# izhengfan/se2lam

Hardware: NVIDIA H100
Metric: ORB keypoints/sec at 640x480 (8-level pyramid, 1000 kps/frame) (higher is better)
Workload: dtype u8

## Files before the change

### se2lam_b200/csrc/fast_screen.h

```cpp
#pragma once
#include <cstdint>

#if defined(__CUDACC__)
#define SE2_HD __host__ __device__ __forceinline__
#else
#define SE2_HD inline
#endif

namespace fastpx {
SE2_HD int16_t lo16(unsigned a) { return (int16_t)(a & 0xFFFF); }
SE2_HD int16_t hi16(unsigned a) { return (int16_t)(a >> 16); }
SE2_HD unsigned pack16(int lo, int hi) { return ((unsigned)lo & 0xFFFFu) | ((unsigned)hi << 16); }
SE2_HD unsigned perm(unsigned a, unsigned b, unsigned s) {
#if defined(__CUDA_ARCH__)
    return __byte_perm(a, b, s);
#else
    const uint64_t src = ((uint64_t)b << 32) | a;
    unsigned r = 0;
    for (int i = 0; i < 4; ++i) {
        const unsigned sel = (s >> (4 * i)) & 0xF;
        unsigned byte = (unsigned)(src >> (8 * (sel & 7))) & 0xFF;
        if (sel & 8) byte = (byte & 0x80) ? 0xFF : 0x00;
        r |= byte << (8 * i);
    }
    return r;
#endif
}
SE2_HD unsigned maxs2(unsigned a, unsigned b) {
#if defined(__CUDA_ARCH__)
    return __vmaxs2(a, b);
#else
    return pack16(lo16(a) > lo16(b) ? lo16(a) : lo16(b), hi16(a) > hi16(b) ? hi16(a) : hi16(b));
#endif
}
SE2_HD unsigned mins2(unsigned a, unsigned b) {
#if defined(__CUDA_ARCH__)
    return __vmins2(a, b);
#else
    return pack16(lo16(a) < lo16(b) ? lo16(a) : lo16(b), hi16(a) < hi16(b) ? hi16(a) : hi16(b));
#endif
}
SE2_HD unsigned min3s2(unsigned a, unsigned b, unsigned c) {
#if defined(__CUDA_ARCH__)
    return __vimin3_s16x2(a, b, c);
#else
    return mins2(mins2(a, b), c);
#endif
}
SE2_HD unsigned max3s2(unsigned a, unsigned b, unsigned c) {
#if defined(__CUDA_ARCH__)
    return __vimax3_s16x2(a, b, c);
#else
    return maxs2(maxs2(a, b), c);
#endif
}
SE2_HD unsigned add2(unsigned a, unsigned b) {
#if defined(__CUDA_ARCH__)
    return __vadd2(a, b);
#else
    return pack16((lo16(a) + lo16(b)) & 0xFFFF, (hi16(a) + hi16(b)) & 0xFFFF);
#endif
}
}

namespace fastpx {

SE2_HD unsigned screen_T1(int t) { return (unsigned)(0x10000 - (257 + t)) * 0x10001u; }
SE2_HD unsigned screen_U1(int t) { return (unsigned)(256 - t) * 0x10001u; }

SE2_HD unsigned screen4(unsigned n3, unsigned s3, unsigned n2l, unsigned n2c, unsigned n2r, unsigned s2l, unsigned s2c, unsigned s2r,
                        unsigned zl, unsigned zc, unsigned zr, unsigned T1, unsigned U1) {
    const unsigned w_m3 = perm(zl, zc, 0x4321), w_p3 = perm(zc, zr, 0x6543);
    const unsigned nw_ = perm(n2l, n2c, 0x5432), ne_ = perm(n2c, n2r, 0x5432);
    const unsigned sw_ = perm(s2l, s2c, 0x5432), se_ = perm(s2c, s2r, 0x5432);
    unsigned m = 0;
#if defined(__CUDA_ARCH__)
#pragma unroll
#endif
    for (int hlf = 0; hlf < 2; ++hlf) {
        const unsigned sel = hlf ? 0x4342u : 0x4140u;
        const unsigned cb = perm(zc, 0, sel) + 0x01000100u;
        const unsigned e0 = cb - perm(s3, 0, sel), e8 = cb - perm(n3, 0, sel);
        const unsigned e4 = cb - perm(w_p3, 0, sel), e12 = cb - perm(w_m3, 0, sel);
        const unsigned e2 = cb - perm(se_, 0, sel), e10 = cb - perm(nw_, 0, sel);
        const unsigned e6 = cb - perm(ne_, 0, sel), e14 = cb - perm(sw_, 0, sel);
        const unsigned D = mins2(min3s2(maxs2(e0, e8), maxs2(e4, e12), maxs2(e2, e10)), maxs2(e6, e14));
        const unsigned B = maxs2(max3s2(mins2(e0, e8), mins2(e4, e12), mins2(e2, e10)), mins2(e6, e14));
        const unsigned r = maxs2(add2(D, T1), add2(~B, U1));
        const unsigned ok = ~r & 0x80008000u;
        m |= ((ok >> 15) & 1u) << (2 * hlf) | ((ok >> 31) & 1u) << (2 * hlf + 1);
    }
    return m;
}

SE2_HD unsigned inside_mask8(int x0, int cw) {
    const int lo = x0 < 0 ? -x0 : 0;
    const int hi = cw - x0 < 8 ? cw - x0 : 8;
    return (0xFFu << lo) & (0xFFu >> (8 - hi)) & 0xFFu;
}

SE2_HD int first_group(int shift) { return (shift + 3) >> 2; }
SE2_HD int groups_per_row(int cw, int shift) { return ((shift + 2 + cw) >> 2) - first_group(shift) + 1; }
SE2_HD int group_x0(int g, int shift) { return 4 * (g + first_group(shift)) - 3 - shift; }
struct ItemWalk {
    int y, g, dY, dG, G;
    SE2_HD void init(int tid, int nthreads, int groups) { G = groups; y = tid / G; g = tid - y * G; dY = nthreads / G; dG = nthreads - dY * G; }
    SE2_HD void next() { g += dG; y += dY; if (g >= G) { g -= G; ++y; } }
};

constexpr int NMS_X0 = 4;
SE2_HD int nms_plane_bytes(int pw, int ch) { return pw * (ch + 2) + 32; }
SE2_HD int nms_words_per_row(int cw) { return (cw + 31) >> 5; }
SE2_HD unsigned nms_row_mask(int k, int cw) { const int n = cw - 32 * k; return n >= 32 ? 0xFFFFFFFFu : (1u << n) - 1u; }

SE2_HD unsigned nms32(const uint32_t* u, const uint32_t* c, const uint32_t* d) {
    unsigned c3e[10], c3o[10];
    unsigned r[4];
#if defined(__CUDA_ARCH__)
#pragma unroll
#endif
    for (int j = 0; j < 10; ++j) {
        const unsigned ua = u[j], ca = c[j], da = d[j];
        if (j > 0) c3e[j] = max3s2(perm(ua, 0, 0x4240), perm(ca, 0, 0x4240), perm(da, 0, 0x4240));
        if (j < 9) c3o[j] = max3s2(perm(ua, 0, 0x4341), perm(ca, 0, 0x4341), perm(da, 0, 0x4341));
    }
#if defined(__CUDA_ARCH__)
#pragma unroll
#endif
    for (int g = 0; g < 8; ++g) {
        const int j = g + 1;
        const unsigned ua = u[j], ca = c[j], da = d[j];
        const unsigned ce = perm(ca, 0, 0x4240), co = perm(ca, 0, 0x4341);
        const unsigned ve = maxs2(perm(ua, 0, 0x4240), perm(da, 0, 0x4240));
        const unsigned vo = maxs2(perm(ua, 0, 0x4341), perm(da, 0, 0x4341));
        const unsigned ne = max3s2(perm(c3o[j - 1], c3o[j], 0x5432), ve, c3o[j]);
        const unsigned no = max3s2(c3e[j], vo, perm(c3e[j], c3e[j + 1], 0x5432));
        const unsigned te = ce + 0x00FF00FFu - ne, to = co + 0x00FF00FFu - no;
        const unsigned bytes = perm(te, to, 0x7351);
        if (g & 1) {
            r[g >> 1] = (r[g >> 1] + (bytes << 4)) * 0x01020408u;
        } else {
            r[g >> 1] = bytes;
        }
    }
    return perm(perm(r[0], r[1], 0x7373), perm(r[2], r[3], 0x7373), 0x5410);
}

struct WordRun {
    int w, w1, y, k, wpr;
    SE2_HD void init(int tid, int nthreads, int ch, int words_per_row) {
        wpr = words_per_row;
        const int nw = ch * wpr, q = (nw + nthreads - 1) / nthreads;
        w = tid * q < nw ? tid * q : nw;
        w1 = w + q < nw ? w + q : nw;
        y = w / wpr; k = w - y * wpr;
    }
    SE2_HD bool more() const { return w < w1; }
    SE2_HD void next() { ++w; if (++k == wpr) { k = 0; ++y; } }
};

}
```

### se2lam_b200/csrc/orb.cu

```cuda
#include <cuda.h>

#include <algorithm>
#include <cmath>
#include <cstring>
#include <type_traits>
#include <vector>

#include "blur_px.h"
#include "common.h"
#include "fast_screen.h"
#include "introselect.h"
#include "resp_key.h"

namespace {

using se2gpu::fail;

constexpr int EDGE = 16;
constexpr int HALF_PATCH = 15;
constexpr int PATCH = 31;
constexpr int MAX_LEVELS = 16;
constexpr int FAST_THREADS = 256;
constexpr int ORB_LANES = 4;
constexpr int BLUR_WARPS = 4;
// ... 24 lines not shown
    int skipped;
    int cand_off, cand_cap;
};

struct TileGeo { int level, strip, cg; };

struct CellHdr { int n_base, n_a, n_b, pad; };

struct OrbDev {
    int nlevels, nfeatures, fast_th, t_lo;
    int n_cells, n_tiles;
    const LevelGeo* levels;
    const CellGeo* cells;
    const TileGeo* tiles;
    const int* itab;
    const short* stab;
    uint8_t* plain;
    uint8_t* blurred;
    size_t frame_plane_bytes;
    uint32_t* cand;
    size_t cand_total;
    CellHdr* hdr;
    uint32_t* lkp;
    int lkp_total;
    int* lcount;
    int* err;
    int frame0;
};

__device__ __forceinline__ int reflect101(int p, int len) {
    if (len == 1) return 0;
    while (p < 0 || p >= len) p = p < 0 ? -p : 2 * (len - 1) - p;
    return p;
}

constexpr int PYR0_ROWS = 4;
__global__ void __launch_bounds__(256) orb_pyr0(OrbDev d, LevelGeo L, const uint8_t* __restrict__ imgs, int stride, size_t frame_stride, int nvec) {
    const int tid = threadIdx.y * 64 + threadIdx.x;
    const int f = blockIdx.z + d.frame0;
    const uint8_t* img = imgs + f * frame_stride;
    uint8_t* plane = d.plain + f * d.frame_plane_bytes + L.plane_off;
    const int rows = L.h + 2 * EDGE;
    if (blockIdx.x + 1 < gridDim.x) {
        const int vx = blockIdx.x * 64 + threadIdx.x;
        const int y0 = (blockIdx.y * 4 + threadIdx.y) * PYR0_ROWS;
        if (vx >= nvec) return;
        uint4 v[PYR0_ROWS];
#pragma unroll
        for (int k = 0; k < PYR0_ROWS; ++k)
            if (y0 + k < rows) v[k] = __ldg(reinterpret_cast<const uint4*>(img + (size_t)reflect101(y0 + k - EDGE, L.h) * stride) + vx);
#pragma unroll
        for (int k = 0; k < PYR0_ROWS; ++k)
            if (y0 + k < rows) *reinterpret_cast<uint4*>(plane + (size_t)(y0 + k) * L.pitch + EDGE + 16 * vx) = v[k];
        return;
    }
    const int tail0 = EDGE + 16 * nvec, nw = 4 + (L.pitch - tail0) / 4;
    for (int item = tid; item < 4 * PYR0_ROWS * nw; item += 256) {
        const int r = item / nw, wi = item - r * nw;
        const int y = blockIdx.y * 4 * PYR0_ROWS + r;
        if (y >= rows) break;
        const int x0 = wi < 4 ? 4 * wi : tail0 + 4 * (wi - 4);
        const uint8_t* row = img + (size_t)reflect101(y - EDGE, L.h) * stride;
        uint32_t word = 0;
#pragma unroll
        for (int q = 0; q < 4; ++q) {
            const int x = x0 + q;
            const uint32_t px = (x < L.w + 2 * EDGE) ? row[reflect101(x - EDGE, L.w)] : 0u;
            word |= px << (8 * q);
        }
        *reinterpret_cast<uint32_t*>(plane + (size_t)y * L.pitch + x0) = word;
    }
}

__global__ void __launch_bounds__(128) orb_pyr0_undistort(OrbDev d, LevelGeo L, const uint8_t* __restrict__ imgs, int stride, size_t frame_stride,
                                                          const short2* __restrict__ m1, const uint16_t* __restrict__ m2) {
    const int x4 = (blockIdx.x * 128 + threadIdx.x) * 4, y = blockIdx.y;
    const int f = blockIdx.z + d.frame0;
    if (x4 >= L.pitch) return;
    const uint8_t* img = imgs + f * frame_stride;
    const int dy = reflect101(y - EDGE, L.h);
    uint32_t word = 0;
#pragma unroll
    for (int q = 0; q < 4; ++q) {
        const int x = x4 + q;
        uint32_t o = 0;
        if (x < L.w + 2 * EDGE) {
            const int idx = dy * L.w + reflect101(x - EDGE, L.w);
            const short2 s = __ldg(m1 + idx);
            const int fr = __ldg(m2 + idx), a = fr & 31, b = fr >> 5;
            const int sx = s.x, sy = s.y;
            const bool x0 = (unsigned)sx < (unsigned)L.w, x1 = (unsigned)(sx + 1) < (unsigned)L.w;
            const bool y0 = (unsigned)sy < (unsigned)L.h, y1 = (unsigned)(sy + 1) < (unsigned)L.h;
            const uint8_t* p = img + (ptrdiff_t)sy * stride + sx;
            const int t00 = (x0 && y0) ? p[0] : 0, t01 = (x1 && y0) ? p[1] : 0, t10 = (x0 && y1) ? p[stride] : 0, t11 = (x1 && y1) ? p[stride + 1] : 0;
            const int val = t00 * ((32 - a) * (32 - b) * 32) + t01 * (a * (32 - b) * 32) + t10 * ((32 - a) * b * 32) + t11 * (a * b * 32);
            o = (uint32_t)min(max((val + (1 << 14)) >> 15, 0), 255);
        }
        word |= o << (8 * q);
    }
    uint8_t* plane = d.plain + f * d.frame_plane_bytes + L.plane_off;
    *reinterpret_cast<uint32_t*>(plane + (size_t)y * L.pitch + x4) = word;
}

constexpr int RESIZE_TR = 32, RESIZE_TR_TALL = 64;
struct ResizeRow { int s0, s1, b0, b1; };
struct ResizeCol { int sx0, sx1; short a0, a1; int valid; };
template <int RESIZE_TR>
__global__ void __launch_bounds__(256) orb_resize_w(OrbDev d, LevelGeo L, LevelGeo S, int max_rows, int raw_pitch) {
    static_assert(RESIZE_TR % 32 == 0 && RESIZE_TR <= 128, "row terms take one thread per row in warps 4..7");
    asm volatile("griddepcontrol.launch_dependents;" ::: "memory");
    extern __shared__ __align__(16) uint8_t rs_smem[];
    __shared__ ResizeRow rowinfo[RESIZE_TR];
    __shared__ __align__(16) ResizeCol colinfo[128];
    __shared__ int s_lo[RESIZE_TR / 32], s_hi[RESIZE_TR / 32];
    __shared__ int s_cmin[4], s_cmax[4];
    uint16_t* hbuf = reinterpret_cast<uint16_t*>(rs_smem);
    uint8_t* raw = rs_smem + (size_t)max_rows * 128 * sizeof(uint16_t);
    const int tx = threadIdx.x, ty = threadIdx.y, tid = ty * 32 + tx;
    const int x4 = blockIdx.x * 128 + tx * 4, y0 = blockIdx.y * RESIZE_TR;
    const int f = blockIdx.z + d.frame0;
    const int W = L.w + 2 * EDGE, H = L.h + 2 * EDGE;
    const int* xofs = d.itab + L.tab_off;
    const int* yofs = xofs + L.w;
    const short2* ialpha = reinterpret_cast<const short2*>(d.stab + 2 * (size_t)L.tab_off);
    const short2* ibeta = ialpha + L.w;
    if (tid < 128) {
        const int x = blockIdx.x * 128 + tid;
        ResizeCol c{0, 0, 0, 0, 0};
        int cmin = 0x7fffffff, cmax = -1;
        if (x < W) {
            const int dx = reflect101(x - EDGE, L.w);
            c.sx0 = __ldg(xofs + dx);
            c.sx1 = min(c.sx0 + 1, S.w - 1);
            const short2 aa = __ldg(ialpha + dx);
            c.a0 = aa.x; c.a1 = aa.y; c.valid = 1;
            cmin = c.sx0; cmax = c.sx1;
        }
        colinfo[tid] = c;
#pragma unroll
        for (int o = 16; o > 0; o >>= 1) { cmin = min(cmin, __shfl_xor_sync(0xffffffffu, cmin, o)); cmax = max(cmax, __shfl_xor_sync(0xffffffffu, cmax, o)); }
        if (tx == 0) { s_cmin[ty] = cmin; s_cmax[ty] = cmax; }
    } else if (ty < 4 + RESIZE_TR / 32) {
        const int ry = tid - 128, y = y0 + ry;
        int rmin = 0x7fffffff, rmax = -1;
        if (y < H) {
            const int dy = reflect101(y - EDGE, L.h);
            const int sy = __ldg(yofs + dy);
            const short2 bb = __ldg(ibeta + dy);
            ResizeRow r{min(max(sy, 0), S.h - 1), min(max(sy + 1, 0), S.h - 1), bb.x, bb.y};
            rowinfo[ry] = r;
            rmin = r.s0; rmax = r.s1;
        }
#pragma unroll
        for (int o = 16; o > 0; o >>= 1) { rmin = min(rmin, __shfl_xor_sync(0xffffffffu, rmin, o)); rmax = max(rmax, __shfl_xor_sync(0xffffffffu, rmax, o)); }
        if (tx == 0) { s_lo[ty - 4] = rmin; s_hi[ty - 4] = rmax; }
    }
    __syncthreads();
    const int c_min = min(min(s_cmin[0], s_cmin[1]), min(s_cmin[2], s_cmin[3])), c_max = max(max(s_cmax[0], s_cmax[1]), max(s_cmax[2], s_cmax[3]));
    const int c_lo = c_min & ~15, nvec = c_max < 0 ? 0 : (c_max - c_lo) / 16 + 1;
    int r_lo = s_lo[0], r_hi = s_hi[0];
#pragma unroll
    for (int k = 1; k < RESIZE_TR / 32; ++k) { r_lo = min(r_lo, s_lo[k]); r_hi = max(r_hi, s_hi[k]); }
    const int nsr = r_hi - r_lo + 1;
    if (nsr > max_rows || nvec * 16 > raw_pitch) { if (tid == 0) *d.err = 3; return; }
    const uint8_t* src = d.plain + f * d.frame_plane_bytes + S.plane_off + (size_t)EDGE * S.pitch + EDGE;
    asm volatile("griddepcontrol.wait;" ::: "memory");
    if (nvec <= 16) {
        const int v = tid & 15;
        if (v < nvec)
            for (int r = tid >> 4; r < nsr; r += 16)
                *reinterpret_cast<uint4*>(raw + r * raw_pitch + 16 * v) = __ldg(reinterpret_cast<const uint4*>(src + (size_t)(r_lo + r) * S.pitch + c_lo) + v);
    } else {
        for (int i = tid; i < nsr * nvec; i += 256) {
            const int r = i / nvec, v = i - r * nvec;
            *reinterpret_cast<uint4*>(raw + r * raw_pitch + 16 * v) = __ldg(reinterpret_cast<const uint4*>(src + (size_t)(r_lo + r) * S.pitch + c_lo) + v);
        }
    }
    int sx0[4], sx1[4], a0[4], a1[4];
    unsigned vmask = 0;
#pragma unroll
    for (int q = 0; q < 4; ++q) {
        const ResizeCol c = colinfo[4 * tx + q];
        sx0[q] = c.valid ? c.sx0 - c_lo : 0; sx1[q] = c.valid ? c.sx1 - c_lo : 0;
        a0[q] = c.a0; a1[q] = c.a1;
        vmask |= c.valid ? (0xFFu << (8 * q)) : 0u;
    }
    __syncthreads();
    unsigned wq[4], selq[4];
    bool pairq[4];
    int w0 = 0;
    bool window_ok = true;
    {
        int mn = 0x7fffffff;
#pragma unroll
        for (int q = 0; q < 4; ++q) if ((vmask >> (8 * q)) & 1u) mn = min(mn, sx0[q]);
        if (mn == 0x7fffffff) mn = 0;
        w0 = mn >> 2;
#pragma unroll
        for (int q = 0; q < 4; ++q) {
            const bool valid = (vmask >> (8 * q)) & 1u;
            const int o = valid ? sx0[q] - 4 * w0 : 0;
            if (valid && (o + 1 > 11 || (sx1[q] != sx0[q] + 1 && a1[q] != 0))) window_ok = false;
            pairq[q] = o >= 7;
            const int o2 = o - (pairq[q] ? 4 : 0);
            selq[q] = (unsigned)o2 | ((unsigned)(o2 + 1) << 4);
            wq[q] = ((unsigned)a0[q] & 0xFFFFu) | ((unsigned)a1[q] << 16);
            if (a0[q] < 0 || a1[q] < 0) window_ok = false;
        }
    }
    if (x4 < W) {
        if (window_ok) {
            for (int r = ty; r < nsr; r += 8) {
                const uint32_t* rw = reinterpret_cast<const uint32_t*>(raw + r * raw_pitch) + w0;
                const uint32_t W0 = rw[0], W1 = rw[1], W2 = rw[2];
                unsigned hq[4];
#pragma unroll
                for (int q = 0; q < 4; ++q) {
                    const unsigned bytes = __byte_perm(pairq[q] ? W1 : W0, pairq[q] ? W2 : W1, selq[q]);
                    hq[q] = __dp2a_lo(wq[q], bytes, 0u) >> 4;
                }
                *reinterpret_cast<uint2*>(hbuf + r * 128 + 4 * tx) = make_uint2(hq[0] | (hq[1] << 16), hq[2] | (hq[3] << 16));
            }
        } else {
            for (int r = ty; r < nsr; r += 8) {
                const uint8_t* rp = raw + r * raw_pitch;
                const unsigned h0 = (unsigned)((rp[sx0[0]] * a0[0] + rp[sx1[0]] * a1[0]) >> 4), h1 = (unsigned)((rp[sx0[1]] * a0[1] + rp[sx1[1]] * a1[1]) >> 4);
                const unsigned h2 = (unsigned)((rp[sx0[2]] * a0[2] + rp[sx1[2]] * a1[2]) >> 4), h3 = (unsigned)((rp[sx0[3]] * a0[3] + rp[sx1[3]] * a1[3]) >> 4);
                *reinterpret_cast<uint2*>(hbuf + r * 128 + 4 * tx) = make_uint2((h0 & 0xFFFFu) | (h1 << 16), (h2 & 0xFFFFu) | (h3 << 16));
            }
        }
    }
    __syncthreads();
    if (x4 >= L.pitch) return;
    uint8_t* plane = d.plain + f * d.frame_plane_bytes + L.plane_off;
#pragma unroll
    for (int k = 0; k < RESIZE_TR / 8; ++k) {
        const int r = ty + 8 * k, y = y0 + r;
        if (y >= H) break;
        uint32_t word = 0;
        if (x4 < W) {
            const ResizeRow ri = rowinfo[r];
            const uint2 A = *reinterpret_cast<const uint2*>(hbuf + (ri.s0 - r_lo) * 128 + 4 * tx);
            const uint2 B = *reinterpret_cast<const uint2*>(hbuf + (ri.s1 - r_lo) * 128 + 4 * tx);
            const unsigned v0 = (unsigned)((((ri.b0 * (int)(A.x & 0xFFFFu)) >> 16) + ((ri.b1 * (int)(B.x & 0xFFFFu)) >> 16) + 2) >> 2);
            const unsigned v1 = (unsigned)((((ri.b0 * (int)(A.x >> 16)) >> 16) + ((ri.b1 * (int)(B.x >> 16)) >> 16) + 2) >> 2);
            const unsigned v2 = (unsigned)((((ri.b0 * (int)(A.y & 0xFFFFu)) >> 16) + ((ri.b1 * (int)(B.y & 0xFFFFu)) >> 16) + 2) >> 2);
            const unsigned v3 = (unsigned)((((ri.b0 * (int)(A.y >> 16)) >> 16) + ((ri.b1 * (int)(B.y >> 16)) >> 16) + 2) >> 2);
            word = (v0 | (v1 << 8) | (v2 << 16) | (v3 << 24)) & vmask;
        }
        *reinterpret_cast<uint32_t*>(plane + (size_t)y * L.pitch + x4) = word;
    }
}

__device__ __forceinline__ unsigned fast_cv(int v) { return (unsigned)(256 + v) | ((unsigned)(256 - v) << 16); }
__device__ __forceinline__ unsigned fast_q(unsigned p, unsigned cv) { return p * 0xFFFFu + cv; }

__device__ __forceinline__ int fast_arc_score(const uint8_t* __restrict__ p, int pw) {
    const unsigned cv = fast_cv(p[0]);
    unsigned q[16];
    q[0] = fast_q(p[3 * pw], cv);       q[1] = fast_q(p[3 * pw + 1], cv);   q[2] = fast_q(p[2 * pw + 2], cv);    q[3] = fast_q(p[pw + 3], cv);
    q[4] = fast_q(p[3], cv);            q[5] = fast_q(p[-pw + 3], cv);      q[6] = fast_q(p[-2 * pw + 2], cv);   q[7] = fast_q(p[-3 * pw + 1], cv);
    q[8] = fast_q(p[-3 * pw], cv);      q[9] = fast_q(p[-3 * pw - 1], cv);  q[10] = fast_q(p[-2 * pw - 2], cv);  q[11] = fast_q(p[-pw - 3], cv);
    q[12] = fast_q(p[-3], cv);          q[13] = fast_q(p[pw - 3], cv);      q[14] = fast_q(p[2 * pw - 2], cv);   q[15] = fast_q(p[3 * pw - 1], cv);
    unsigned m3[16];
#pragma unroll
    for (int k = 0; k < 16; ++k) m3[k] = __vimin3_s16x2(q[k], q[(k + 1) & 15], q[(k + 2) & 15]);
    unsigned best = 0;
#pragma unroll
    for (int k = 0; k < 16; k += 2) {
        const unsigned a9 = __vimin3_s16x2(m3[k], m3[(k + 3) & 15], m3[(k + 6) & 15]);
        const unsigned b9 = __vimin3_s16x2(m3[k + 1], m3[(k + 4) & 15], m3[(k + 7) & 15]);
        best = __vimax3_s16x2(best, a9, b9);
    }
    return (int)max(best & 0xFFFFu, best >> 16) - 256;
}

struct FastMaps { CUtensorMap m[MAX_LEVELS]; };
__device__ __forceinline__ unsigned orb_smem_u32(const void* p) { return (unsigned)__cvta_generic_to_shared(p); }
__device__ __forceinline__ void orb_mbar_init(unsigned long long* bar, unsigned count) {
    asm volatile("mbarrier.init.shared::cta.b64 [%0], %1;" ::"r"(orb_smem_u32(bar)), "r"(count) : "memory");
    asm volatile("fence.mbarrier_init.release.cluster;" ::: "memory");
}
__device__ __forceinline__ bool orb_mbar_wait(unsigned long long* bar, unsigned parity) {
    const long long t0 = clock64();
    for (;;) {
        unsigned done;
        asm volatile(
            "{\n"
            ".reg .pred p;\n"
            "mbarrier.try_wait.parity.shared::cta.b64 p, [%1], %2;\n"
            "selp.u32 %0, 1, 0, p;\n"
            "}\n" : "=r"(done) : "r"(orb_smem_u32(bar)), "r"(parity) : "memory");
        if (done) return true;
        if (clock64() - t0 > 400000000LL) return false;
    }
}
__device__ __forceinline__ void orb_tma_box3(void* dst_smem, const CUtensorMap* map, int x, int y, int z, unsigned bytes, unsigned long long* bar) {
    asm volatile("mbarrier.arrive.expect_tx.shared::cta.b64 _, [%0], %1;" ::"r"(orb_smem_u32(bar)), "r"(bytes) : "memory");
    asm volatile("cp.async.bulk.tensor.3d.shared::cluster.global.tile.mbarrier::complete_tx::bytes [%0], [%1, {%2, %3, %4}], [%5];"
                 ::"r"(orb_smem_u32(dst_smem)), "l"(map), "r"(x), "r"(y), "r"(z), "r"(orb_smem_u32(bar)) : "memory");
}

template <bool TMA>
__global__ void __launch_bounds__(FAST_THREADS, TMA ? 0 : 5) orb_fast_cells(OrbDev d, const __grid_constant__ FastMaps maps) {
    extern __shared__ __align__(128) uint8_t smem_raw[];
    __shared__ int s_ncand, s_wsum[FAST_THREADS / 32];
    __shared__ __align__(8) unsigned long long s_bar;
    const CellGeo c = d.cells[blockIdx.x];
    const int f = blockIdx.y + d.frame0;
    CellHdr* hdr = d.hdr + (size_t)f * d.n_cells + blockIdx.x;
    const int cw = c.x1 - c.x0, ch = c.y1 - c.y0;
    if (c.skipped || cw <= 0 || ch <= 0) {
        if (threadIdx.x == 0) { hdr->n_base = 0; hdr->n_a = 0; hdr->n_b = 0; }
        return;
    }
    const LevelGeo& L = d.levels[c.level];
    const int bx0 = c.x0 - 3 + EDGE, ax0 = bx0 & (TMA ? ~15 : ~3), shift = bx0 - ax0;
    const int pw = TMA ? L.fbw : (shift + cw + 6 + 3) & ~3, pww = pw >> 2;
    const int ph = TMA ? L.fbh : ch + 6;
    uint8_t* smem = TMA ? smem_raw + ((128u - (orb_smem_u32(smem_raw) & 127u)) & 127u) : smem_raw;
    const int g0 = fastpx::first_group(shift), G = fastpx::groups_per_row(cw, shift), nitems = ch * G;
    const int wpr = fastpx::nms_words_per_row(cw);
    uint8_t* patch = smem;
    uint8_t* score = smem + ((pw * ph + 15) & ~15);
    uint32_t* bitmap = reinterpret_cast<uint32_t*>(score + ((fastpx::nms_plane_bytes(pw, ch) + 15) & ~15));
    uint16_t* list = reinterpret_cast<uint16_t*>(bitmap + ch * wpr);
    if (TMA) {
        if (threadIdx.x == 0) orb_mbar_init(&s_bar, 1);
        __syncthreads();
        if (threadIdx.x == 0) orb_tma_box3(patch, &maps.m[c.level], ax0, c.y0 - 3 + EDGE, f, (unsigned)(pw * ph), &s_bar);
    } else {
        const uint8_t* plane = d.plain + f * d.frame_plane_bytes + L.plane_off;
        const int by0 = c.y0 - 3 + EDGE;
        for (int i = threadIdx.x; i < pww * ph; i += FAST_THREADS) {
            const int py = i / pww, pxw = i - py * pww;
            reinterpret_cast<uint32_t*>(patch)[i] = *reinterpret_cast<const uint32_t*>(plane + (size_t)(by0 + py) * L.pitch + ax0 + 4 * pxw);
        }
    }
    constexpr int NW = FAST_THREADS / 32;
    const int lane = threadIdx.x & 31, wid = threadIdx.x >> 5;
    const uint8_t* p0 = patch + 3 * pw + 3 + shift;
    fastpx::ItemWalk first;
    first.init((int)threadIdx.x, FAST_THREADS, G);
    fastpx::WordRun words;
    words.init((int)threadIdx.x, FAST_THREADS, ch, wpr);
    int thr = d.fast_th;
    int total = 0, pos0 = 0;
    for (int pass = 0; pass < 2; ++pass) {
        for (int i = threadIdx.x; i < pw * (ch + 2) / 4; i += FAST_THREADS) reinterpret_cast<uint32_t*>(score)[i] = 0u;
        if (threadIdx.x == 0) s_ncand = 0;
        if (TMA && pass == 0 && !orb_mbar_wait(&s_bar, 0)) { *d.err = 4; return; }
        __syncthreads();
        {
            const uint32_t* pwords = reinterpret_cast<const uint32_t*>(patch);
            const unsigned T1 = fastpx::screen_T1(thr), U1 = fastpx::screen_U1(thr);
            fastpx::ItemWalk it = first;
            for (int it0 = wid * 32; it0 < nitems; it0 += NW * 32) {
                unsigned m = 0;
                const int col0 = fastpx::group_x0(it.g, shift);
                if (it.y < ch) {
                    const uint32_t* c = pwords + (it.y + 3) * pww + it.g + g0;
                    const uint32_t n3 = c[-3 * pww], s3 = c[3 * pww];
                    const uint32_t n2a = c[-2 * pww - 1], n2b = c[-2 * pww], n2c = c[-2 * pww + 1];
                    const uint32_t s2a = c[2 * pww - 1], s2b = c[2 * pww], s2c = c[2 * pww + 1];
                    const uint32_t za = c[-1], zb = c[0], zc = c[1];
                    m = fastpx::screen4(n3, s3, n2a, n2b, n2c, s2a, s2b, s2c, za, zb, zc, T1, U1) & fastpx::inside_mask8(col0, cw) & 0xFu;
                }
                const unsigned b0 = __ballot_sync(0xffffffffu, m & 1u), b1 = __ballot_sync(0xffffffffu, m & 2u);
                const unsigned b2 = __ballot_sync(0xffffffffu, m & 4u), b3 = __ballot_sync(0xffffffffu, m & 8u);
                const int n0 = __popc(b0), n01 = n0 + __popc(b1), n012 = n01 + __popc(b2), tot = n012 + __popc(b3);
                if (tot) {
                    int base = 0;
                    if (lane == 0) base = atomicAdd(&s_ncand, tot);
                    base = __shfl_sync(0xffffffffu, base, 0);
                    const unsigned lt = (1u << lane) - 1u;
                    const int e0 = it.y * pw + col0;
                    if (m & 1u) list[base + __popc(b0 & lt)] = (uint16_t)e0;
                    if (m & 2u) list[base + n0 + __popc(b1 & lt)] = (uint16_t)(e0 + 1);
                    if (m & 4u) list[base + n01 + __popc(b2 & lt)] = (uint16_t)(e0 + 2);
                    if (m & 8u) list[base + n012 + __popc(b3 & lt)] = (uint16_t)(e0 + 3);
                }
                it.next();
            }
        }
        __syncthreads();
        const int ncand = s_ncand;
        for (int i = threadIdx.x; i < ncand; i += FAST_THREADS) {
            const int off = list[i];
            const int m = fast_arc_score(p0 + off, pw);
            if (m > thr) score[off + pw + fastpx::NMS_X0] = (uint8_t)(m - 1);
        }
        __syncthreads();
        int nkp = 0;
        for (fastpx::WordRun r = words; r.more(); r.next()) {
            const uint32_t* u = reinterpret_cast<const uint32_t*>(score) + r.y * pww + 8 * r.k;
            const unsigned bits = fastpx::nms32(u, u + pww, u + 2 * pww) & fastpx::nms_row_mask(r.k, cw);
            bitmap[r.w] = bits;
            nkp += __popc(bits);
        }
        int inc = nkp;
#pragma unroll
        for (int o = 1; o < 32; o <<= 1) { const int u = __shfl_up_sync(0xffffffffu, inc, o); if (lane >= o) inc += u; }
        if (lane == 31) s_wsum[wid] = inc;
        __syncthreads();
        total = 0; pos0 = inc - nkp;
#pragma unroll
        for (int w = 0; w < NW; ++w) { const int v = s_wsum[w]; total += v; if (w < wid) pos0 += v; }
        if (total > 3 || thr == 7) break;
        thr = 7;
    }
    uint32_t* out = d.cand + (size_t)f * d.cand_total + c.cand_off;
    int pos = pos0;
    for (fastpx::WordRun r = words; r.more(); r.next()) {
        uint32_t bits = bitmap[r.w];
        const uint8_t* srow = score + (r.y + 1) * pw + fastpx::NMS_X0 + 32 * r.k;
        const uint32_t yx = ((uint32_t)(c.y0 + r.y) << 12) | (uint32_t)(c.x0 + 32 * r.k);
        while (bits) {
            const int i = __ffs(bits) - 1;
            bits &= bits - 1;
            if (pos < c.cand_cap) out[pos] = ((uint32_t)srow[i] << 24) | (yx + i);
            else *d.err = 1;
            ++pos;
        }
    }
    if (threadIdx.x == 0) { hdr->n_base = total; hdr->n_a = total; hdr->n_b = total; }
}

__device__ __forceinline__ int fast_arc_score_qr(const uint8_t* __restrict__ p, int pw, int t) {
    const int v = p[0];
    const int c0 = v - p[3 * pw], c8 = v - p[-3 * pw];
    bool dk = (c0 > t) | (c8 > t), br = (c0 < -t) | (c8 < -t);
    if (!(dk | br)) return 0;
    const int c4 = v - p[3], c12 = v - p[-3];
    dk &= (c4 > t) | (c12 > t); br &= (c4 < -t) | (c12 < -t);
    if (!(dk | br)) return 0;
    const int c2 = v - p[2 * pw + 2], c10 = v - p[-2 * pw - 2];
    dk &= (c2 > t) | (c10 > t); br &= (c2 < -t) | (c10 < -t);
    if (!(dk | br)) return 0;
    const int c6 = v - p[-2 * pw + 2], c14 = v - p[2 * pw - 2];
    dk &= (c6 > t) | (c14 > t); br &= (c6 < -t) | (c14 < -t);
    if (!(dk | br)) return 0;
#define SE2_PK(dv) ((static_cast<unsigned>(dv) & 0xFFFFu) | (static_cast<unsigned>(-(dv)) << 16))
    unsigned q[16];
    q[0] = SE2_PK(c0);   q[1] = SE2_PK(v - p[3 * pw + 1]);    q[2] = SE2_PK(c2);    q[3] = SE2_PK(v - p[pw + 3]);
    q[4] = SE2_PK(c4);   q[5] = SE2_PK(v - p[-pw + 3]);       q[6] = SE2_PK(c6);    q[7] = SE2_PK(v - p[-3 * pw + 1]);
    q[8] = SE2_PK(c8);   q[9] = SE2_PK(v - p[-3 * pw - 1]);   q[10] = SE2_PK(c10);  q[11] = SE2_PK(v - p[-pw - 3]);
    q[12] = SE2_PK(c12); q[13] = SE2_PK(v - p[pw - 3]);       q[14] = SE2_PK(c14);  q[15] = SE2_PK(v - p[3 * pw - 1]);
#undef SE2_PK
    unsigned m3[16];
#pragma unroll
    for (int k = 0; k < 16; ++k) m3[k] = __vimin3_s16x2(q[k], q[(k + 1) & 15], q[(k + 2) & 15]);
    unsigned best = 0x80008000u;
#pragma unroll
    for (int k = 0; k < 16; k += 2) {
        const unsigned a9 = __vimin3_s16x2(m3[k], m3[(k + 3) & 15], m3[(k + 6) & 15]);
        const unsigned b9 = __vimin3_s16x2(m3[k + 1], m3[(k + 4) & 15], m3[(k + 7) & 15]);
        best = __vimax3_s16x2(best, a9, b9);
    }
    const int mdark = static_cast<short>(best & 0xFFFFu), mbright = static_cast<short>(best >> 16);
    return max(mdark, mbright);
}

__global__ void __launch_bounds__(FAST_THREADS) orb_fast_cells_big(OrbDev d) {
    extern __shared__ uint8_t smem[];
    __shared__ int s_total;
    const CellGeo c = d.cells[blockIdx.x];
    const int f = blockIdx.y + d.frame0;
    CellHdr* hdr = d.hdr + (size_t)f * d.n_cells + blockIdx.x;
    const int cw = c.x1 - c.x0, ch = c.y1 - c.y0;
    if (c.skipped || cw <= 0 || ch <= 0) {
        if (threadIdx.x == 0) { hdr->n_base = 0; hdr->n_a = 0; hdr->n_b = 0; }
        return;
    }
    const LevelGeo& L = d.levels[c.level];
    const uint8_t* plane = d.plain + f * d.frame_plane_bytes + L.plane_off;
    const int bx0 = c.x0 - 3 + EDGE, by0 = c.y0 - 3 + EDGE;
    const int ax0 = bx0 & ~3, shift = bx0 - ax0;
    const int ph = ch + 6, sw = cw + 2, sh = ch + 2;
    const int pww = (shift + cw + 6 + 3) >> 2, pw = pww * 4;
    uint8_t* patch = smem;
    uint8_t* score = smem + ((pw * ph + 15) & ~15);
    const int nseg = (cw + 31) >> 5, nchunk = ch * nseg;
    int* cnt = reinterpret_cast<int*>(score + ((sw * sh + 15) & ~15));
    for (int i = threadIdx.x; i < pww * ph; i += FAST_THREADS) {
        const int py = i / pww, pxw = i - py * pww;
        reinterpret_cast<uint32_t*>(patch)[i] = *reinterpret_cast<const uint32_t*>(plane + (size_t)(by0 + py) * L.pitch + ax0 + 4 * pxw);
    }
    constexpr int NW = FAST_THREADS / 32;
    const int lane = threadIdx.x & 31, wid = threadIdx.x >> 5;
    const uint8_t* p0 = patch + 3 * pw + 3 + shift;
    int thr = d.fast_th;
    unsigned long long keepmask = 0;
    for (int pass = 0; pass < 2; ++pass) {
        for (int i = threadIdx.x; i < (sw * sh + 3) / 4; i += FAST_THREADS) reinterpret_cast<uint32_t*>(score)[i] = 0u;
        __syncthreads();
        for (int cidx = wid; cidx < nchunk; cidx += NW) {
            const int y = cidx / nseg, x = (cidx - y * nseg) * 32 + lane;
            if (x < cw) {
                const int m = fast_arc_score_qr(p0 + y * pw + x, pw, thr);
                if (m > thr) score[(y + 1) * sw + (x + 1)] = (uint8_t)(m - 1);
            }
        }
        __syncthreads();
        keepmask = 0;
        int t = 0;
        for (int cidx = wid; cidx < nchunk; cidx += NW, ++t) {
            const int y = cidx / nseg, x = (cidx - y * nseg) * 32 + lane;
            bool keep = false;
            if (x < cw) {
                const uint8_t* q = score + (y + 1) * sw + (x + 1);
                const int s = q[0];
                if (s) keep = s > q[-sw - 1] && s > q[-sw] && s > q[-sw + 1] && s > q[-1] && s > q[1] && s > q[sw - 1] && s > q[sw] && s > q[sw + 1];
            }
            const unsigned bal = __ballot_sync(0xffffffffu, keep);
            if (lane == 0) cnt[cidx] = __popc(bal);
            if (keep && t < 64) keepmask |= 1ull << t;
        }
        __syncthreads();
        if (wid == 0) {
            int run = 0;
            for (int b0 = 0; b0 < nchunk; b0 += 32) {
                const int v = (b0 + lane < nchunk) ? cnt[b0 + lane] : 0;
                int inc = v;
#pragma unroll
                for (int o = 1; o < 32; o <<= 1) { const int u = __shfl_up_sync(0xffffffffu, inc, o); if (lane >= o) inc += u; }
                if (b0 + lane < nchunk) cnt[b0 + lane] = run + inc - v;
                run += __shfl_sync(0xffffffffu, inc, 31);
            }
            if (lane == 0) s_total = run;
        }
        __syncthreads();
        if (s_total > 3 || thr == 7) break;
        thr = 7;
        __syncthreads();
    }
    uint32_t* out = d.cand + (size_t)f * d.cand_total + c.cand_off;
    int t = 0;
    for (int cidx = wid; cidx < nchunk; cidx += NW, ++t) {
        const int y = cidx / nseg, x = (cidx - y * nseg) * 32 + lane;
        bool keep;
        int s = 0;
        if (t < 64) {
            keep = (keepmask >> t) & 1ull;
        } else {
            keep = false;
            if (x < cw) {
                const uint8_t* q = score + (y + 1) * sw + (x + 1);
                s = q[0];
                if (s) keep = s > q[-sw - 1] && s > q[-sw] && s > q[-sw + 1] && s > q[-1] && s > q[1] && s > q[sw - 1] && s > q[sw] && s > q[sw + 1];
            }
        }
        const unsigned bal = __ballot_sync(0xffffffffu, keep);
        if (keep) {
            s = score[(y + 1) * sw + (x + 1)];
            const int pos = cnt[cidx] + __popc(bal & ((1u << lane) - 1));
            if (pos < c.cand_cap) out[pos] = ((uint32_t)s << 24) | ((uint32_t)(c.y0 + y) << 12) | (uint32_t)(c.x0 + x);
            else *d.err = 1;
        }
    }
    if (threadIdx.x == 0) { hdr->n_base = s_total; hdr->n_a = s_total; hdr->n_b = s_total; }
}

constexpr int HARRIS_THREADS = 128;
constexpr float HARRIS_SCALE = 1.0f / ((1 << 2) * 7 * 255.0f);
constexpr float HARRIS_SCALE_SQ_SQ = HARRIS_SCALE * HARRIS_SCALE * HARRIS_SCALE * HARRIS_SCALE;
__global__ void __launch_bounds__(HARRIS_THREADS) orb_harris(OrbDev d, uint64_t* __restrict__ cand64) {
    const CellGeo c = d.cells[blockIdx.x];
    const int f = blockIdx.y + d.frame0;
    if (c.skipped) return;
    const int n = min(d.hdr[(size_t)f * d.n_cells + blockIdx.x].n_base, c.cand_cap);
    if (n <= 0) return;
    const LevelGeo& L = d.levels[c.level];
    const uint8_t* plane = d.plain + f * d.frame_plane_bytes + L.plane_off;
    const size_t co = (size_t)f * d.cand_total + c.cand_off;
    const uint32_t* cand = d.cand + co;
    for (int i = threadIdx.x; i < n; i += HARRIS_THREADS) {
        const uint32_t rec = cand[i];
        const int x = rec & 0xFFF, y = (rec >> 12) & 0xFFF;
        const int bx = EDGE + x - 4, ax = bx & ~3;
        const unsigned sh = 8u * (unsigned)(bx - ax);
        const uint8_t* row0 = plane + (size_t)(EDGE + y - 4) * L.pitch + ax;
        int p[9][9];
#pragma unroll
        for (int r = 0; r < 9; ++r) {
            const uint32_t* w = reinterpret_cast<const uint32_t*>(row0 + (size_t)r * L.pitch);
            const uint32_t w0 = __ldg(w), w1 = __ldg(w + 1), w2 = __ldg(w + 2);
            const uint32_t lo = __funnelshift_r(w0, w1, sh), mid = __funnelshift_r(w1, w2, sh), hi = __funnelshift_r(w2, 0u, sh);
#pragma unroll
            for (int k = 0; k < 4; ++k) { p[r][k] = __byte_perm(lo, 0u, 0x4440 + k); p[r][4 + k] = __byte_perm(mid, 0u, 0x4440 + k); }
            p[r][8] = hi & 0xFF;
        }
        int a = 0, b = 0, cc = 0;
#pragma unroll
        for (int r = 1; r < 8; ++r)
#pragma unroll
            for (int k = 1; k < 8; ++k) {
                const int Ix = (p[r][k + 1] - p[r][k - 1]) * 2 + (p[r - 1][k + 1] - p[r - 1][k - 1]) + (p[r + 1][k + 1] - p[r + 1][k - 1]);
                const int Iy = (p[r + 1][k] - p[r - 1][k]) * 2 + (p[r + 1][k - 1] - p[r - 1][k - 1]) + (p[r + 1][k + 1] - p[r - 1][k + 1]);
                a += Ix * Ix; b += Iy * Iy; cc += Ix * Iy;
            }
        const float fa = __int2float_rn(a), fb = __int2float_rn(b), fc = __int2float_rn(cc);
        const float apb = __fadd_rn(fa, fb);
        const float t = __fsub_rn(__fsub_rn(__fmul_rn(fa, fb), __fmul_rn(fc, fc)), __fmul_rn(__fmul_rn(0.04f, apb), apb));
        const float resp = __fmul_rn(t, HARRIS_SCALE_SQ_SQ);
        cand64[co + i] = ((uint64_t)se2gpu::resp_key(resp) << 32) | rec;
    }
}

constexpr int SEL_STAGE = 12288;
constexpr int SEL_THREADS = 512;
struct HarrisBufs { uint64_t* cand64; float* lresp; };
template <bool HARRIS>
__global__ void __launch_bounds__(SEL_THREADS) orb_select(OrbDev d, HarrisBufs hb) {
    typedef typename std::conditional<HARRIS, se2gpu::KpKey64, se2gpu::KpScore32>::type K;
    typedef typename K::rec R;
    constexpr int STAGE = HARRIS ? SEL_STAGE / 2 : SEL_STAGE;
    extern __shared__ uint32_t sbuf[];
    __shared__ int wq[SEL_THREADS / 32][128];
    constexpr int NW = SEL_THREADS / 32;
    const int lane = threadIdx.x & 31, wid = threadIdx.x >> 5;
    const int level = blockIdx.x, f = blockIdx.y + d.frame0;
    const LevelGeo& L = d.levels[level];
    const int nCells = L.nCells;
    const int cap = 2 * L.nDesired + 4 * nCells + 64;
    R* lbuf = reinterpret_cast<R*>(sbuf);
    int* nTotal = (int*)(lbuf + cap);
    int* nToRetain = nTotal + nCells;
    int* kept = nToRetain + nCells;
    int* koff = kept + nCells;
    R* stage = (R*)(koff + nCells);
    __shared__ int s_total, s_staged;
    const CellHdr* hdr = d.hdr + (size_t)f * d.n_cells + L.cell_base;
    R* cand;
    if constexpr (HARRIS) cand = hb.cand64 + (size_t)f * d.cand_total;
    else cand = d.cand + (size_t)f * d.cand_total;
    for (int c = threadIdx.x; c < nCells; c += SEL_THREADS) nTotal[c] = d.cells[L.cell_base + c].skipped ? 0 : hdr[c].n_base;
    __syncthreads();
    if (threadIdx.x == 0) {
        const int nfeaturesCell = L.nfeaturesCell;
        int nNoMore = 0, nToDistribute = 0, tot = 0;
        for (int c = 0; c < nCells; ++c) {
            const bool skipped = d.cells[L.cell_base + c].skipped;
            koff[c] = 0;
            tot += nTotal[c];
            if (skipped) { nToRetain[c] = 0; continue; }
            if (nTotal[c] > nfeaturesCell) nToRetain[c] = nfeaturesCell;
            else { nToRetain[c] = nTotal[c]; nToDistribute += nfeaturesCell - nTotal[c]; koff[c] = 1; nNoMore++; }
        }
        while (nToDistribute > 0 && nNoMore < nCells) {
            const int nNew = (int)((float)nfeaturesCell + ceilf((float)nToDistribute / (float)(nCells - nNoMore)));
            nToDistribute = 0;
            for (int c = 0; c < nCells; ++c)
                if (!koff[c]) {
                    if (nTotal[c] > nNew) nToRetain[c] = nNew;
                    else { nToRetain[c] = nTotal[c]; nToDistribute += nNew - nTotal[c]; koff[c] = 1; nNoMore++; }
                }
        }
        s_staged = tot <= STAGE;
        int o = 0;
        for (int c = 0; c < nCells; ++c) { kept[c] = o; o += nTotal[c]; }
    }
    __syncthreads();
    const bool staged = s_staged;
    for (int c = wid; c < nCells; c += NW) {
        const int n = nToRetain[c], tot = nTotal[c];
        R* g = cand + d.cells[L.cell_base + c].cand_off;
        R* v = g;
        if (staged) {
            v = stage + kept[c];
            for (int i = lane; i < tot; i += 32) v[i] = g[i];
            __syncwarp();
        }
        if (lane == 0) koff[c] = (int)(v - (staged ? stage : cand));
        if (tot > n && n > 0) se2gpu::kp_nth_element_warp<K>(v, tot, n - 1, wq[wid]);
    }
    __syncthreads();
    if (threadIdx.x == 0) {
        int o = 0;
        for (int c = 0; c < nCells; ++c) { const int k = min(nTotal[c], nToRetain[c]); nTotal[c] = k; kept[c] = o; o += k; }
        if (o > cap) { *d.err = 2; o = cap; }
        s_total = o;
    }
    __syncthreads();
    for (int c = wid; c < nCells; c += NW) {
// ... 965 lines not shown
```

Measured before the change: 103.4 million.

## Screen eight pixels per thread, simplify FAST test, use per-thread atomic list append

Each screening item now covers two 4-pixel groups (8 pixels), sharing neighbor word loads between them. The FAST pre-screen is rewritten to compare raw ring pixels against the centre with a single bias constant rather than computing per-pixel differences. The warp-ballot compaction is replaced by a per-thread shared atomicAdd followed by a sequential append, and the TMA kernel now gets a min-blocks launch bound of 5. The candidate list order becomes nondeterministic, and per-thread shared atomics may contend more than the old one-atomic-per-warp scheme.

```diff
diff --git a/se2lam_b200/csrc/fast_screen.h b/se2lam_b200/csrc/fast_screen.h
--- a/se2lam_b200/csrc/fast_screen.h
+++ b/se2lam_b200/csrc/fast_screen.h
@@ -65,32 +65,36 @@
 
 namespace fastpx {
 
-SE2_HD unsigned screen_T1(int t) { return (unsigned)(0x10000 - (257 + t)) * 0x10001u; }
-SE2_HD unsigned screen_U1(int t) { return (unsigned)(256 - t) * 0x10001u; }
+SE2_HD unsigned screen_bias(int t) { return (unsigned)(511 - t) * 0x10001u; }
 
 SE2_HD unsigned screen4(unsigned n3, unsigned s3, unsigned n2l, unsigned n2c, unsigned n2r, unsigned s2l, unsigned s2c, unsigned s2r,
-                        unsigned zl, unsigned zc, unsigned zr, unsigned T1, unsigned U1) {
+                        unsigned zl, unsigned zc, unsigned zr, unsigned bias) {
     const unsigned w_m3 = perm(zl, zc, 0x4321), w_p3 = perm(zc, zr, 0x6543);
     const unsigned nw_ = perm(n2l, n2c, 0x5432), ne_ = perm(n2c, n2r, 0x5432);
     const unsigned sw_ = perm(s2l, s2c, 0x5432), se_ = perm(s2c, s2r, 0x5432);
-    unsigned m = 0;
+    unsigned ok[2];
 #if defined(__CUDA_ARCH__)
 #pragma unroll
 #endif
     for (int hlf = 0; hlf < 2; ++hlf) {
-        const unsigned sel = hlf ? 0x4342u : 0x4140u;
-        const unsigned cb = perm(zc, 0, sel) + 0x01000100u;
-        const unsigned e0 = cb - perm(s3, 0, sel), e8 = cb - perm(n3, 0, sel);
-        const unsigned e4 = cb - perm(w_p3, 0, sel), e12 = cb - perm(w_m3, 0, sel);
-        const unsigned e2 = cb - perm(se_, 0, sel), e10 = cb - perm(nw_, 0, sel);
-        const unsigned e6 = cb - perm(ne_, 0, sel), e14 = cb - perm(sw_, 0, sel);
-        const unsigned D = mins2(min3s2(maxs2(e0, e8), maxs2(e4, e12), maxs2(e2, e10)), maxs2(e6, e14));
-        const unsigned B = maxs2(max3s2(mins2(e0, e8), mins2(e4, e12), mins2(e2, e10)), mins2(e6, e14));
-        const unsigned r = maxs2(add2(D, T1), add2(~B, U1));
-        const unsigned ok = ~r & 0x80008000u;
-        m |= ((ok >> 15) & 1u) << (2 * hlf) | ((ok >> 31) & 1u) << (2 * hlf + 1);
+        const unsigned sel = hlf ? 0x4341u : 0x4240u;
+        const unsigned v = perm(zc, 0, sel);
+        const unsigned p0 = perm(s3, 0, sel), p8 = perm(n3, 0, sel);
+        const unsigned p4 = perm(w_p3, 0, sel), p12 = perm(w_m3, 0, sel);
+        const unsigned p2 = perm(se_, 0, sel), p10 = perm(nw_, 0, sel);
+        const unsigned p6 = perm(ne_, 0, sel), p14 = perm(sw_, 0, sel);
+        const unsigned lo = maxs2(max3s2(mins2(p0, p8), mins2(p4, p12), mins2(p2, p10)), mins2(p6, p14));
+        const unsigned hi = mins2(min3s2(maxs2(p0, p8), maxs2(p4, p12), maxs2(p2, p10)), maxs2(p6, p14));
+        ok[hlf] = ((v + bias - lo) | (hi + bias - v)) & 0x02000200u;
     }
-    return m;
+    const unsigned b = ok[0] + (ok[1] << 1);
+    return ((b >> 9) | (b >> 23)) & 0xFu;
+}
+SE2_HD unsigned screen_T1(int t) { return screen_bias(t); }
+SE2_HD unsigned screen_U1(int t) { return screen_bias(t); }
+SE2_HD unsigned screen4(unsigned n3, unsigned s3, unsigned n2l, unsigned n2c, unsigned n2r, unsigned s2l, unsigned s2c, unsigned s2r,
+                        unsigned zl, unsigned zc, unsigned zr, unsigned T1, unsigned ) {
+    return screen4(n3, s3, n2l, n2c, n2r, s2l, s2c, s2r, zl, zc, zr, T1);
 }
 
 SE2_HD unsigned inside_mask8(int x0, int cw) {
@@ -102,6 +106,7 @@
 SE2_HD int first_group(int shift) { return (shift + 3) >> 2; }
 SE2_HD int groups_per_row(int cw, int shift) { return ((shift + 2 + cw) >> 2) - first_group(shift) + 1; }
 SE2_HD int group_x0(int g, int shift) { return 4 * (g + first_group(shift)) - 3 - shift; }
+SE2_HD int items_per_row(int cw, int shift) { return (groups_per_row(cw, shift) + 1) >> 1; }
 struct ItemWalk {
     int y, g, dY, dG, G;
     SE2_HD void init(int tid, int nthreads, int groups) { G = groups; y = tid / G; g = tid - y * G; dY = nthreads / G; dG = nthreads - dY * G; }
diff --git a/se2lam_b200/csrc/orb.cu b/se2lam_b200/csrc/orb.cu
--- a/se2lam_b200/csrc/orb.cu
+++ b/se2lam_b200/csrc/orb.cu
@@ -350,7 +350,7 @@
 }
 
 template <bool TMA>
-__global__ void __launch_bounds__(FAST_THREADS, TMA ? 0 : 5) orb_fast_cells(OrbDev d, const __grid_constant__ FastMaps maps) {
+__global__ void __launch_bounds__(FAST_THREADS, 5) orb_fast_cells(OrbDev d, const __grid_constant__ FastMaps maps) {
     extern __shared__ __align__(128) uint8_t smem_raw[];
     __shared__ int s_ncand, s_wsum[FAST_THREADS / 32];
     __shared__ __align__(8) unsigned long long s_bar;
@@ -367,7 +367,7 @@
     const int pw = TMA ? L.fbw : (shift + cw + 6 + 3) & ~3, pww = pw >> 2;
     const int ph = TMA ? L.fbh : ch + 6;
     uint8_t* smem = TMA ? smem_raw + ((128u - (orb_smem_u32(smem_raw) & 127u)) & 127u) : smem_raw;
-    const int g0 = fastpx::first_group(shift), G = fastpx::groups_per_row(cw, shift), nitems = ch * G;
+    const int g0 = fastpx::first_group(shift), G = fastpx::items_per_row(cw, shift), nitems = ch * G;
     const int wpr = fastpx::nms_words_per_row(cw);
     uint8_t* patch = smem;
     uint8_t* score = smem + ((pw * ph + 15) & ~15);
@@ -401,33 +401,25 @@
         __syncthreads();
         {
             const uint32_t* pwords = reinterpret_cast<const uint32_t*>(patch);
-            const unsigned T1 = fastpx::screen_T1(thr), U1 = fastpx::screen_U1(thr);
+            const unsigned bias = fastpx::screen_bias(thr);
             fastpx::ItemWalk it = first;
             for (int it0 = wid * 32; it0 < nitems; it0 += NW * 32) {
                 unsigned m = 0;
-                const int col0 = fastpx::group_x0(it.g, shift);
+                const int col0 = fastpx::group_x0(2 * it.g, shift);
                 if (it.y < ch) {
-                    const uint32_t* c = pwords + (it.y + 3) * pww + it.g + g0;
-                    const uint32_t n3 = c[-3 * pww], s3 = c[3 * pww];
-                    const uint32_t n2a = c[-2 * pww - 1], n2b = c[-2 * pww], n2c = c[-2 * pww + 1];
-                    const uint32_t s2a = c[2 * pww - 1], s2b = c[2 * pww], s2c = c[2 * pww + 1];
-                    const uint32_t za = c[-1], zb = c[0], zc = c[1];
-                    m = fastpx::screen4(n3, s3, n2a, n2b, n2c, s2a, s2b, s2c, za, zb, zc, T1, U1) & fastpx::inside_mask8(col0, cw) & 0xFu;
+                    const uint32_t* c = pwords + (it.y + 3) * pww + 2 * it.g + g0;
+                    const uint32_t n3a = c[-3 * pww], n3b = c[-3 * pww + 1], s3a = c[3 * pww], s3b = c[3 * pww + 1];
+                    const uint32_t n2a = c[-2 * pww - 1], n2b = c[-2 * pww], n2c = c[-2 * pww + 1], n2d = c[-2 * pww + 2];
+                    const uint32_t s2a = c[2 * pww - 1], s2b = c[2 * pww], s2c = c[2 * pww + 1], s2d = c[2 * pww + 2];
+                    const uint32_t za = c[-1], zb = c[0], zc = c[1], zd = c[2];
+                    m = (fastpx::screen4(n3a, s3a, n2a, n2b, n2c, s2a, s2b, s2c, za, zb, zc, bias) |
+                         fastpx::screen4(n3b, s3b, n2b, n2c, n2d, s2b, s2c, s2d, zb, zc, zd, bias) << 4) & fastpx::inside_mask8(col0, cw);
                 }
-                const unsigned b0 = __ballot_sync(0xffffffffu, m & 1u), b1 = __ballot_sync(0xffffffffu, m & 2u);
-                const unsigned b2 = __ballot_sync(0xffffffffu, m & 4u), b3 = __ballot_sync(0xffffffffu, m & 8u);
-                const int n0 = __popc(b0), n01 = n0 + __popc(b1), n012 = n01 + __popc(b2), tot = n012 + __popc(b3);
-                if (tot) {
-                    int base = 0;
-                    if (lane == 0) base = atomicAdd(&s_ncand, tot);
-                    base = __shfl_sync(0xffffffffu, base, 0);
-                    const unsigned lt = (1u << lane) - 1u;
-                    const int e0 = it.y * pw + col0;
-                    if (m & 1u) list[base + __popc(b0 & lt)] = (uint16_t)e0;
-                    if (m & 2u) list[base + n0 + __popc(b1 & lt)] = (uint16_t)(e0 + 1);
-                    if (m & 4u) list[base + n01 + __popc(b2 & lt)] = (uint16_t)(e0 + 2);
-                    if (m & 8u) list[base + n012 + __popc(b3 & lt)] = (uint16_t)(e0 + 3);
-                }
+                uint16_t* dst = list + atomicAdd(&s_ncand, __popc(m));
+                const int e0 = it.y * pw + col0;
+#pragma unroll
+                for (int j = 0; j < 8; ++j)
+                    if (m & (1u << j)) *dst++ = (uint16_t)(e0 + j);
                 it.next();
             }
         }
```

Result: faster. 109.4 million (median of 6 runs) (+5.9%).
